# kostastsa/BayesianFiltering

Measured on AMD Instinct MI355X. Metric: filter timesteps/sec (batch x T), higher is better.
Workload: dtype f32; 1 GPU; batched Kalman filter state_dim=4 obs_dim=2 T=10000 batch=65536 per GPU, K=1, all five posterior streams (FULL5), layout=reference, observations drawn from the model; batch_per_gpu=65536, T=10000, state_dim=4, obs_dim=2, parallelism=batch-sharded x1

## Files before the change

bayesianfiltering_amd/csrc/bf_api.hip:

```cpp
#include <cstring>
#include "bf_common.hpp"
#include "../../include/bayesfilt_ext2.h"
#include "forward_host.hpp"
#include "pscan_host.hpp"
#include "user_model.hpp"
#include "bf_rng.hpp"

namespace bf {

char* last_error_buf() {
  static thread_local char buf[512] = {0};
  return buf;
}

int set_error(int code, const char* fmt, ...) {
  va_list ap;
  va_start(ap, fmt);
  vsnprintf(last_error_buf(), 512, fmt, ap);
  va_end(ap);
  return code;
}

int launch_kf_group(const bf_lgssm* p, const bf_cstream* y, long long B, long long T, const bf_carry* carry,
                    const bf_out_desc* out, hipStream_t stream, int force_mode, int lanes);
// ... 56 lines not shown
static Option g_kf_lanes{0, OPT_KF_LANES};
__host__ __device__ inline float canon_eval_one(int op, const float* in, long long n, long long i) {
  const float x = in[i];
  float s, c;
  switch (op) {
    case 0: return canon_log(x);
    case 1: return canon_exp(x);
    case 2: return bits_to_normal(canon_f_bits(x));
    case 3: canon_sincos(x, &s, &c); return s;
    case 4: canon_sincos(x, &s, &c); return c;
    default: return canon_atan2(x, in[n + i]);
  }
}
__global__ void canon_eval_kernel(int op, const float* __restrict__ in, long long n, float* __restrict__ out) {
  const long long i = (long long)blockIdx.x * blockDim.x + threadIdx.x;
  if (i >= n) return;
  out[i] = canon_eval_one(op, in, n, i);
}

Option& rts_load_mode_option();
static Option g_kf_small_mode{1, OPT_KF_SMALL_MODE};
static Option g_force_generic{0, OPT_FORCE_GENERIC};
Option& force_generic_option() { return g_force_generic; }

static bool kf_small_tiles(int n, int m) { return n >= 9 && n <= 32 && m <= 32 && (n >= 16 || m > 8) && g_kf_small_mode.load() != 0; }

struct GsfTiles {
  bool linear;
  bf_lgssm lg;
  int dyn_kind;
  float dth[8];
};
static GsfTiles gsf_tiles(const bf_model* model, int K) {
  GsfTiles t;
  std::memset(&t, 0, sizeof(t));
  const bool lin_emi = model->emi_id == 0 && model->n_emi_theta == model->m * model->n + model->m * model->dr;
  const bool lin_dyn = model->dyn_id == 0 && model->n_dyn_theta == model->n * model->n + model->n * model->dq;
  t.dyn_kind = (model->dyn_id == 1 && model->n_dyn_theta == 5 && model->dq == model->n) ? 1
             : (model->dyn_id == 4 && model->n_dyn_theta == 1 && model->dq == model->n) ? 2 : 0;
  t.linear = lin_emi && model->flags == 0 && K <= 64 && (lin_dyn || t.dyn_kind != 0);
  if (!t.linear) return t;
  bf_lgssm& lg = t.lg;
  lg.n = model->n; lg.dq = model->dq; lg.m = model->m; lg.dr = model->dr;
  if (lin_dyn) { lg.A = model->dyn_theta; lg.G = model->dyn_theta + model->n * model->n; t.dyn_kind = 0; }
  lg.H = model->emi_theta; lg.D = model->emi_theta + model->m * model->n;
  lg.q0 = model->q0; lg.r0 = model->r0; lg.Q = model->Q; lg.R = model->R;
  lg.Q_steps = model->Q_steps > 0 ? model->Q_steps : 1; lg.R_steps = model->R_steps > 0 ? model->R_steps : 1;
  if (!lin_dyn) for (int i = 0; i < model->n_dyn_theta && i < 8; ++i) t.dth[i] = model->dyn_theta[i];
  return t;
}
Option& ffbs_spl_option();
Option& pkf_block_option();
Option& prs_block_option();
Option& pfs_block_option();
long long kf_pscan_workspace_bytes(int n, int m, long long B, long long T, int block);
int launch_kf_pscan(const bf_lgssm* model, const bf_cstream* y, long long B, long long T, const bf_carry* carry,
                    const bf_out_desc* out, void* workspace, long long workspace_bytes, hipStream_t stream, bool missing);

template <class F>
static int with_generic_fallback(int rc, F&& generic) {
  if (rc != BF_EUNSUPPORTED) return rc;
  char first[512];
  std::snprintf(first, sizeof(first), "%s", last_error_buf());
  const int rc2 = generic();
  if (rc2 == BF_OK) return BF_OK;
  char second[512];
  std::snprintf(second, sizeof(second), "%s", last_error_buf());
  return set_error(rc2, "%.240s; generic kernel: %.240s", first, second);
}

}

extern "C" {

int bf_version(void) { return BF_VERSION; }

int bf_abi_check(int32_t header_version, size_t sizeof_out_desc, size_t sizeof_lgssm, size_t sizeof_model,
                 size_t sizeof_bpf_model, size_t sizeof_bpf_out) {
  if (header_version / 100 != BF_VERSION / 100)
    return bf::set_error(BF_EINVAL, "binding was written against header version %d, the library is %d", (int)header_version, BF_VERSION);
  BF_ABI_SIZE(sizeof_out_desc, bf_out_desc)
  BF_ABI_SIZE(sizeof_lgssm, bf_lgssm)
  BF_ABI_SIZE(sizeof_model, bf_model)
  BF_ABI_SIZE(sizeof_bpf_model, bf_bpf_model)
  BF_ABI_SIZE(sizeof_bpf_out, bf_bpf_out)
  return BF_OK;
}

const char* bf_last_error(void) { return bf::last_error_buf(); }

int bf_device_count(void) {
  int n = 0;
  if (hipGetDeviceCount(&n) != hipSuccess) return 0;
  int ok = 0;
  for (int i = 0; i < n; ++i) {
    hipDeviceProp_t prop;
    if (hipGetDeviceProperties(&prop, i) == hipSuccess && std::strncmp(prop.gcnArchName, "gfx950", 6) == 0) ++ok;
  }
  return ok;
}

static int set_option_impl(const char* name, int value, bool this_call_only) {
  struct Row {
    const char* name;
    bf::Option& option;
    bool (*accept)(int);
    const char* message;
  };
  const auto flag = [](int v) { return v == 0 || v == 1; };
  const auto pscan_block = [](int v) { return v == 0 || (v >= bf::PSCAN_L_MIN && v <= bf::PSCAN_L_MAX); };
  static_assert(bf::PSCAN_L_MIN == 4 && bf::PSCAN_L_MAX == 4096, "the *_block messages below spell the limits out");
  const Row rows[] = {
      {"kf_emit_mode", bf::g_kf_emit_mode, [](int v) { return v >= -1 && v <= 2; }, "kf_emit_mode must be -1..2"},
      {"kf_lanes", bf::g_kf_lanes, [](int v) { return v >= 0 && v <= 64 && (v & (v - 1)) == 0; }, "kf_lanes must be 0 or a power of two <= 64"},
      {"kf_small_mode", bf::g_kf_small_mode, flag, "kf_small_mode must be 0 or 1"},
      {"force_generic", bf::g_force_generic, flag, "force_generic must be 0 or 1"},
      {"ugsf_force_generic", bf::g_ugsf_force_generic, flag, "ugsf_force_generic must be 0 or 1"},
      {"agsf_force_generic", bf::g_agsf_force_generic, flag, "agsf_force_generic must be 0 or 1"},
      {"rts_load_mode", bf::rts_load_mode_option(), [](int v) { return v == -1 || v == 0 || v == 2; }, "rts_load_mode must be -1, 0 or 2"},
      {"ffbs_spl", bf::ffbs_spl_option(), [](int v) { return v == 0 || v == 1 || v == 2 || v == 4 || v == 8; }, "ffbs_spl must be 0, 1, 2, 4 or 8"},
      {"pkf_block", bf::pkf_block_option(), pscan_block, "pkf_block must be 0 or 4..4096"},
      {"prs_block", bf::prs_block_option(), pscan_block, "prs_block must be 0 or 4..4096"},
      {"pfs_block", bf::pfs_block_option(), pscan_block, "pfs_block must be 0 or 4..4096"},
      {"gsf_structured", bf::g_gsf_structured, flag, "gsf_structured must be 0 or 1"},
      {"bpf_variant", bf::g_bpf_variant, flag, "bpf_variant must be 0 or 1"},
      {"bpf_hbm_mode", bf::g_bpf_hbm_mode, [](int v) { return v >= 0 && v <= 2; }, "bpf_hbm_mode must be 0, 1 or 2"},
      {"bpf_arith", bf::g_bpf_arith, flag, "bpf_arith must be 0 or 1"},
      {"bpf_spec", bf::g_bpf_spec, flag, "bpf_spec must be 0 or 1"},
  };
  for (const Row& r : rows) {
    if (!name || std::strcmp(name, r.name) != 0) continue;
    if (!r.accept(value)) return bf::set_error(BF_EINVAL, "%s", r.message);
    if (this_call_only) {
      bf::CallOverrides& c = bf::call_overrides();
      c.value[r.option.id] = value;
      c.armed[r.option.id] = true;
    } else {
      r.option = value;
    }
    return BF_OK;
  }
  return bf::set_error(BF_EINVAL, "unknown option '%s'", name ? name : "(null)");
}

int bf_set_option(const char* name, int value) { return set_option_impl(name, value, false); }

int bf_set_call_option(const char* name, int value) { return set_option_impl(name, value, true); }

int64_t bf_bytes_per_step(int32_t n, int32_t m, int32_t K, const bf_out_desc* out) {
  int64_t per = 0;
  if (!out) {
    per = 1 + 2 * (int64_t)n + 2 * (int64_t)n * n;
  } else {
    if (out->weights.ptr) per += 1;
    if (out->means.ptr) per += n;
    if (out->covs.ptr) per += (int64_t)n * n;
    if (out->pred_means.ptr) per += n;
    if (out->pred_covs.ptr) per += (int64_t)n * n;
    if (out->loglik.ptr) per += 1;
  }
  int64_t once = 0;
  if (out && out->coll_mean.ptr) once += n;
  if (out && out->coll_cov.ptr) once += (int64_t)n * n;
  return 4 * (int64_t)m + 4 * (int64_t)K * per + 4 * once;
}

int bf_kalman_filter_f32(const bf_lgssm* model, const bf_cstream* y, int64_t B, int64_t T, const bf_carry* carry,
                         const bf_out_desc* out, void* stream) {
// ... 333 lines not shown
```

bayesianfiltering_amd/csrc/bf_common.hpp:

```cpp
#pragma once
#include <hip/hip_runtime.h>
#include <cstdarg>
#include <cstdio>
#include <cstdint>
#include <atomic>
#include <iterator>
#include "../../include/bayesfilt.h"
#include "bf_views.hpp"

namespace bf {

char* last_error_buf();
int set_error(int code, const char* fmt, ...);

#define BF_HIP_CHECK(expr)                                                                   \
  do {                                                                                       \
    hipError_t e_ = (expr);                                                                  \
    if (e_ != hipSuccess)                                                                    \
      return ::bf::set_error(BF_EHIP, "%s failed: %s (%s:%d)", #expr, hipGetErrorString(e_), \
                             __FILE__, __LINE__);                                            \
  } while (0)

#define BF_ABI_SIZE(NAME_, T_)           \
  if (NAME_ != 0 && NAME_ != sizeof(T_)) \
    return ::bf::set_error(BF_EINVAL, "binding's sizeof(" #T_ ") = %zu, the library's is %zu: the struct layouts differ", NAME_, sizeof(T_));

enum OptionId { OPT_KF_EMIT_MODE, OPT_KF_LANES, OPT_KF_SMALL_MODE, OPT_FORCE_GENERIC, OPT_GSF_STRUCTURED,
                OPT_BPF_VARIANT, OPT_BPF_HBM_MODE, OPT_BPF_SPEC, OPT_BPF_ARITH, OPT_RTS_LOAD_MODE, OPT_UGSF_FORCE_GENERIC, OPT_FFBS_SPL,
                OPT_AGSF_FORCE_GENERIC, OPT_PKF_BLOCK, OPT_PRS_BLOCK, OPT_PFS_BLOCK,
                OPT_COUNT };
struct CallOverrides {
  int value[OPT_COUNT];
  bool armed[OPT_COUNT];
};
CallOverrides& call_overrides();
struct Option {
  std::atomic<int> global;
  OptionId id;
  Option(int v, OptionId i) : global(v), id(i) {}
  int load() const {
    const CallOverrides& c = call_overrides();
    return c.armed[id] ? c.value[id] : global.load();
  }
  operator int() const { return load(); }
  Option& operator=(int v) {
    global = v;
    return *this;
  }
};
void begin_call_constants();
void release_call_constants();
struct CallOptionScope {
  CallOptionScope() { begin_call_constants(); }
  ~CallOptionScope() {
    CallOverrides& c = call_overrides();
    for (int i = 0; i < OPT_COUNT; ++i) c.armed[i] = false;
    release_call_constants();
  }
};

int device_constants(const void* host, size_t bytes, hipStream_t stream, const void** d_out);

#ifndef BF_MISSING
#define BF_MISSING false
#endif
#if BF_MISSING
#define BF_GROUP_FN(FAMILY_, G_) launch_##FAMILY_##_missing_group_##G_
#else
#define BF_GROUP_FN(FAMILY_, G_) launch_##FAMILY_##_group_##G_
#endif

template <class Group, class... Args>
inline int run_groups(Group* const* groups, size_t count, bool* matched, const Args&... args) {
  *matched = false;
  for (size_t g = 0; g < count; ++g) {
    const int rc = groups[g](args..., matched);
    if (*matched) return rc;
  }
  return BF_OK;
}

inline SView make_sview(const bf_stream& s) { return SView{s.ptr, s.sB, s.sK, s.sT, s.sE}; }
// ... 5 lines not shown
```

bayesianfiltering_amd/csrc/kf_scan_mfma.hip:

```cpp
#include <cstdlib>
#include "forward_host.hpp"
#include "lgssm_pack.hpp"
#include "mfma_multi.hpp"
#include "mfma_tiles.hpp"

namespace bf {

template <int N, int M>
struct MfmaConst {
  float reserved[N * N + M * N];
  float GQG[N * N], DRD[M * M], Gq0[N], Dr0[M];
  float dth[8];
  unsigned short A3[3][N * N], H3[3][M * N];
};

__device__ __attribute__((noinline)) void chol_w_rows_bf(lds_f* sc, lds_f* sT, lds_f* sv, lds_f* mcur, lds_f* mnxt, lds_f* scv, lds_c* wt,
                                                         int lane) {
  chol_w_rows_impl<64>(sc, sT, sv, mcur, mnxt, scv, wt, lane);
}
__device__ __attribute__((noinline, used)) float chol_loglik_rows(lds_f* sc, lds_f* sv, int lane) { return chol_loglik_rows_impl(sc, sv, lane); }

template <int N>
__device__ __forceinline__ void store_tile(const SView& sv, long long b, long long t, int pi, int pj, int lane, const f32x16& acc, int k = 0) {
  if (!sv.p) return;
  const int lr = lane & 31, lk = lane >> 5;
  gl_f* base = per_step(sv.p + b * sv.sB + k * sv.sK + t * sv.sT);
  const unsigned e0 = (unsigned)((32 * pi + 4 * lk) * N + 32 * pj + lr);
  if (sv.sE == 1) {
    BF_UNROLL for (int r = 0; r < 16; ++r) __builtin_nontemporal_store(acc[r], base + (e0 + ((r & 3) + 8 * (r >> 2)) * N));
  } else {
    const long long sE = sv.sE + (long long)opaque_szero();
    const unsigned e0s = e0 + (unsigned)opaque_zero();
    BF_UNROLL for (int r = 0; r < 16; ++r) __builtin_nontemporal_store(acc[r], base + (long long)(e0s + ((r & 3) + 8 * (r >> 2)) * N) * sE);
  }
}
template <int N>
__device__ __forceinline__ void store_tile_n(const SView& sv, long long b, long long t, int pi, int pj, int lane, const f32x16& acc, int nr, int k = 0) {
  if (nr == N) return store_tile<N>(sv, b, t, pi, pj, lane, acc, k);
  if (!sv.p) return;
  const int lr = lane & 31, lk = lane >> 5;
  gl_f* base = per_step(sv.p + b * sv.sB + k * sv.sK + t * sv.sT);
  const int col = 32 * pj + lr;
  const long long sE = sv.sE + (long long)opaque_szero();
  BF_UNROLL for (int r = 0; r < 16; ++r) {
    const int row = 32 * pi + (r & 3) + 8 * (r >> 2) + 4 * lk;
    if (col < nr && row < nr) __builtin_nontemporal_store(acc[r], base + (long long)(row * nr + col) * sE);
  }
}

__device__ __forceinline__ float dot_terms_half(const u32x4 (*x)[4], const float* v, int lk, int h) {
  float s = 0.f;
  BF_UNROLL for (int cc = 0; cc < 2; ++cc) BF_UNROLL for (int d = 0; d < 4; ++d) {
    const u32x4 x0v = h ? x[0][2 + cc] : x[0][cc], x1v = h ? x[1][2 + cc] : x[1][cc], x2v = h ? x[2][2 + cc] : x[2][cc];
    const float x0 = (bf_lo(x0v[d]) + bf_lo(x1v[d])) + bf_lo(x2v[d]);
    const float x1 = (bf_hi(x0v[d]) + bf_hi(x1v[d])) + bf_hi(x2v[d]);
    const int k = 16 * (2 * h + cc) + 8 * lk + 2 * d;
    s = fmaf(x0, v[k], s);
    s = fmaf(x1, v[k + 1], s);
  }
  return s;
}

template <int N, int M, bool MULTI = false, bool TV = false, int DYN = 0>
__global__ void __launch_bounds__(256, 2)
kf_scan_mfma5_kernel(const MfmaConst<N, M>* __restrict__ cst, CView y, CarryView carry, OutViews out, long long B, long long T,
                     int rot_mode, int nr, int mr, int K, const float* __restrict__ tvq, const float* __restrict__ tvr) {
  static_assert(N == 64 && M == 32, "tile assignment is written for n = 64, m = 32");
  constexpr int PS = M + 1, HPP = N + 1;
  constexpr int PITCH = 144, PN_TERM = 64 * PITCH, ZN_TERM = 32 * PITCH, WT_PITCH = 80, WT_TERM = 64 * WT_PITCH;
  constexpr int OFF_ZN = 3 * PN_TERM, OFF_WT = OFF_ZN + 3 * ZN_TERM, OFF_YN = OFF_ZN, OFF_F32 = OFF_WT + 3 * WT_TERM;
  static_assert(3 * PN_TERM <= 3 * ZN_TERM + 3 * WT_TERM, "Y^T aliases Z and W^T");
  const int tid = threadIdx.x;
  const int lane = tid & 63;
  const int lr = lane & 31, lk = lane >> 5;
  __shared__ int s_rot;
  if (tid == 0) {
    const unsigned hw = __builtin_amdgcn_s_getreg((31 << 11) | 4);
    const unsigned k = (hw >> 4) & 3, pos = ((k & 1) << 1) | (k >> 1);
    s_rot = rot_mode == 0 ? (int)blockIdx.x : (int)(pos + 2 * (hw & 15));
  }
  __syncthreads();
  const int wave = __builtin_amdgcn_readfirstlane(((tid >> 6) + s_rot) & 3);
  const int ti = wave >> 1, tj = wave & 1;
  const long long b = blockIdx.x;
  const long long bt = MULTI ? b / K : b;
  const int kc = MULTI ? (int)(b % K) : 0;

  extern __shared__ __attribute__((aligned(16))) float lds[];
  lds_c* L = (lds_c*)reinterpret_cast<char*>(lds);
  lds_c* Pn = L;
  lds_c* Zn = L + OFF_ZN;
  lds_c* Wt = L + OFF_WT;
  lds_c* Yn = L + OFF_YN;
  float* sHP = lds + OFF_F32 / 4;
  float* sc2 = sHP + M * HPP;
  float* sc3 = sc2 + M * PS;
  float* sm = sc3 + M * PS;
  float* sm2 = sm + N;
  float* sv = sm2 + N;
  float* scv = sv + M;
  float* part = scv + N;
  float* sv3 = part + 2 * N;

  u32x4 hop[3][4], aop[3][4];
  BF_UNROLL for (int t = 0; t < 3; ++t) BF_UNROLL for (int c = 0; c < 4; ++c) {
    hop[t][c] = *reinterpret_cast<const u32x4*>(&cst->H3[t][lr * N + 16 * c + 8 * lk]);
    if constexpr (DYN == 0) aop[t][c] = *reinterpret_cast<const u32x4*>(&cst->A3[t][(32 * tj + lr) * N + 16 * c + 8 * lk]);
  }
  f32x16 Pacc;
  const bool col_ok = 32 * tj + lr < nr;
  BF_UNROLL for (int r = 0; r < 16; ++r) {
    const int row = 32 * ti + c_row(r, lane);
    Pacc[r] = (col_ok && row < nr) ? carry.P_in[b * nr * nr + row * nr + 32 * tj + lr] : 0.f;
  }
  store_terms_transposed(Pn, PN_TERM, PITCH, ti, tj, lane, Pacc);
  if (tid < N) sm[tid] = tid < nr ? carry.m_in[b * nr + tid] : 0.f;
  float w = (!MULTI && carry.w_in) ? carry.w_in[b] : 1.0f;
  float ynext = (wave >= 2 && lane < mr) ? y.p[bt * y.sB + lane * y.sE] : 0.f;
  const float ll_pad = 0.5f * 1.8378770664093453f * (float)(M - mr);
  const float dr0 = cst->Dr0[lr], gq0 = cst->Gq0[lane];
  __syncthreads();

#ifdef BF_MFMA_PHASE_TIMERS
  long long tacc[12] = {0};
  long long tprev = wall_clock64();
#define BF_TICK5(i) { const long long tn_ = wall_clock64(); tacc[i] += tn_ - tprev; tprev = tn_; }
#else
#define BF_TICK5(i)
#endif
  float* mcur = sm;
  float* mnxt = sm2;
  for (long long t = 0; t < T; ++t) {
    float yv_t = ynext;
    if (wave >= 2) {
      const long long tn = t + 1 < T ? t + 1 : t;
      if (lane < mr) ynext = y.p[bt * y.sB + tn * y.sT + lane * y.sE];
    }
    gl_cf* const drd_t = TV && tvr ? per_step(tvr + t * (M * M)) : per_step(cst->DRD);
    gl_cf* const gqg_t = TV && tvq ? per_step(tvq + t * (N * N)) : per_step(cst->GQG);
    if (wave < 2) {
      f32x16 z = {0};
      BF_UNROLL for (int c = 0; c < 4; ++c) {
        u32x4 a[3];
        load_terms(a, Pn, PN_TERM, PITCH, 32 * wave + lr, c, lk);
        const u32x4 bh[3] = {hop[0][c], hop[1][c], hop[2][c]};
        z = mfma_bf6(a, bh, z);
      }
      BF_UNROLL for (int r = 0; r < 16; ++r) sHP[lr * HPP + 32 * wave + c_row(r, lane)] = z[r];
      store_terms_transposed(Zn, ZN_TERM, PITCH, wave, 0, lane, z);
    } else {
      float s = dot_terms_half(hop, mcur, lk, wave - 2);
      s += __shfl_xor(s, 32, 64);
      if (lane < M) part[(wave - 2) * N + lane] = s;
    }
    BF_TICK5(0)
    lds_barrier();
    BF_TICK5(1)
    float ll = 0.f;
    if (wave >= 2) {
      {
        if (lane < M) (wave == 2 ? sv : sv3)[lane] = yv_t - ((part[lane] + part[N + lane]) + dr0);
      }
      f32x16 acc;
      BF_UNROLL for (int r = 0; r < 16; ++r) acc[r] = drd_t[lr * M + c_row(r, lane)];
      BF_UNROLL for (int c = 0; c < 4; ++c) {
        u32x4 bz[3];
        load_terms(bz, Zn, ZN_TERM, PITCH, lr, c, lk);
        const u32x4 ah[3] = {hop[0][c], hop[1][c], hop[2][c]};
        acc = mfma_bf6(ah, bz, acc);
      }
      float* sc = wave == 2 ? sc2 : sc3;
      BF_UNROLL for (int r = 0; r < 16; ++r) sc[lr * PS + c_row(r, lane)] = acc[r];
      wave_lds_order();
      BF_TICK5(10)
      if (wave == 3) chol_w_rows_bf((lds_f*)sc3, (lds_f*)sHP, (lds_f*)sv3, (lds_f*)mcur, (lds_f*)mnxt, (lds_f*)scv, Wt, lane);
      else ll = chol_loglik_rows((lds_f*)sc2, (lds_f*)sv, lane) + ll_pad;
    }
    BF_TICK5(2)
    lds_barrier();
    BF_TICK5(3)
    {
      f32x16 acc = Pacc;
      BF_UNROLL for (int c = 0; c < 2; ++c) {
        u32x4 a[3], bw[3];
        load_terms(a, Wt, WT_TERM, WT_PITCH, 32 * ti + lr, c, lk);
        load_terms(bw, Wt, WT_TERM, WT_PITCH, 32 * tj + lr, c, lk);
        BF_UNROLL for (int q = 0; q < 3; ++q) a[q] ^= 0x80008000u;
        acc = mfma_bf6(a, bw, acc);
      }
      acc = mfma2(lk == 0 ? scv[32 * ti + lr] : 0.f, lk == 0 ? scv[32 * tj + lr] : 0.f, acc);
      store_tile_n<N>(out.P, bt, t, ti, tj, lane, acc, nr, kc);
      store_terms_transposed(Pn, PN_TERM, PITCH, ti, tj, lane, acc);
    }
    if (wave == 1 && out.m.p && lane < nr) out.m.p[bt * out.m.sB + kc * out.m.sK + t * out.m.sT + lane * out.m.sE] = mnxt[lane];
    if (wave == 2 && lane == 0) {
      if constexpr (!MULTI) {
        w = reweight_single(ll, w);
        if (out.w.p) out.w.p[b * out.w.sB + t * out.w.sT] = w;
      }
      if (out.ll.p) out.ll.p[bt * out.ll.sB + kc * out.ll.sK + t * out.ll.sT] = ll;
    }
    BF_TICK5(4)
    lds_barrier();
    BF_TICK5(5)
    float gq[16];
    BF_UNROLL for (int r = 0; r < 16; ++r) gq[r] = gqg_t[(32 * ti + c_row(r, lane)) * N + 32 * tj + lr];
    if constexpr (DYN != 0) {
      gl_cf* th = per_step(cst->dth);
      const int row = 32 * tj + lr;
      float fv = 0.f;
      BF_UNROLL for (int c = 0; c < 4; ++c) {
        float fr[8];
        BF_UNROLL for (int e = 0; e < 8; ++e) fr[e] = 0.f;
        if (row < nr) {
          if constexpr (DYN == 1) {
            const float alpha = th[0], beta = th[1], gamma = th[2], dt = th[3];
            const bool mp = th[4] != 0.f;
            const int im1 = (row + nr - 1) % nr, ip1 = (row + 1) % nr, im2 = (row + 2 * nr - 2) % nr;
            const float xi = mnxt[row], ax = mnxt[im1];
            const float bx = mp ? (mnxt[ip1] - mnxt[im2]) : 0.f;
            fv = xi + dt * (alpha * (ax * bx) - beta * xi + gamma);
            BF_UNROLL for (int e = 0; e < 8; ++e) {
              const int j = 16 * c + 8 * lk + e;
              float v = 0.f;
              if (j == row) v += 1.0f - dt * beta;
              if (mp) {
                if (j == im1) v += dt * alpha * bx;
                if (j == ip1) v += dt * alpha * ax;
                if (j == im2) v -= dt * alpha * ax;
              }
              fr[e] = v;
            }
          } else {
            const float w0 = th[0], xi = mnxt[row];
            fv = sinf(w0 * xi);
            const float d = w0 * cosf(w0 * xi);
            BF_UNROLL for (int e = 0; e < 8; ++e) fr[e] = (16 * c + 8 * lk + e == row) ? d : 0.f;
          }
        }
        BF_UNROLL for (int d = 0; d < 4; ++d) {
          const Split3 sp = split_pair(fr[2 * d], fr[2 * d + 1]);
          aop[0][c][d] = sp.hi; aop[1][c][d] = sp.mid; aop[2][c][d] = sp.lo;
        }
      }
      if (ti == 0 && lane < 32) { part[32 * tj + lane] = fv; part[N + 32 * tj + lane] = 0.f; }
    }
    {
      f32x16 acc = {0};
      BF_UNROLL for (int c = 0; c < 4; ++c) {
        u32x4 a[3];
        load_terms(a, Pn, PN_TERM, PITCH, 32 * ti + lr, c, lk);
        const u32x4 ba[3] = {aop[0][c], aop[1][c], aop[2][c]};
        acc = mfma_bf6(a, ba, acc);
      }
      store_terms_transposed(Yn, PN_TERM, PITCH, ti, tj, lane, acc);
    }
    if constexpr (DYN == 0) {
      float s = dot_terms_half(aop, mnxt, lk, ti);
      s += __shfl_xor(s, 32, 64);
      if (lane < 32) part[ti * N + 32 * tj + lane] = s;
    }
    BF_TICK5(6)
    lds_barrier();
    BF_TICK5(7)
    {
      if (wave == 2) mcur[lane] = (part[lane] + part[N + lane]) + gq0;
      BF_UNROLL for (int r = 0; r < 16; ++r) Pacc[r] = 0.f;
      BF_UNROLL for (int c = 0; c < 4; ++c) {
        u32x4 a[3];
        load_terms(a, Yn, PN_TERM, PITCH, 32 * ti + lr, c, lk);
        const u32x4 ba[3] = {aop[0][c], aop[1][c], aop[2][c]};
        Pacc = mfma_bf6(a, ba, Pacc);
      }
      BF_UNROLL for (int r = 0; r < 16; ++r) Pacc[r] += gq[r];
      store_tile_n<N>(out.pP, bt, t, ti, tj, lane, Pacc, nr, kc);
      store_terms_transposed(Pn, PN_TERM, PITCH, ti, tj, lane, Pacc);
    }
    if (wave == 2 && out.pm.p && lane < nr) out.pm.p[bt * out.pm.sB + kc * out.pm.sK + t * out.pm.sT + lane * out.pm.sE] = (part[lane] + part[N + lane]) + gq0;
    BF_TICK5(8)
    lds_barrier();
    BF_TICK5(9)
  }

  if (carry.P_out && col_ok) BF_UNROLL for (int r = 0; r < 16; ++r) {
      const int row = 32 * ti + c_row(r, lane);
      if (row < nr) carry.P_out[b * nr * nr + row * nr + 32 * tj + lr] = Pacc[r];
    }
  if (carry.m_out && tid < nr) carry.m_out[b * nr + tid] = mcur[tid];
  if (!MULTI && carry.w_out && wave == 2 && lane == 0) carry.w_out[b] = w;
#ifdef BF_MFMA_PHASE_TIMERS
  __syncthreads();
  if (b == 0 && lane == 0 && carry.P_out) for (int i = 0; i < 12; ++i) carry.P_out[wave * 16 + i] = (float)tacc[i];
#endif
}

int launch_kf_mfma(const bf_lgssm* p, const bf_cstream* y, long long B, long long T, const bf_carry* carry,
                   const bf_out_desc* out, hipStream_t stream, int K, bool multi, int dyn_kind, const float* dth) {
  constexpr int N = 64, M = 32;
  const int nr = p->n, mr = p->m, dq = p->dq, dr = p->dr;
  if (nr > N || mr > M) return set_error(BF_EUNSUPPORTED, "MFMA Kalman kernel: n <= 64 and m <= 32");
  if (dyn_kind != 0 && (!multi || p->G || dq != nr)) return set_error(BF_EINVAL, "nonlinear chains: identity noise input, multi launch");
  if (K > 64) return set_error(BF_EUNSUPPORTED, "MFMA Kalman kernel: at most 64 components (one per lane in the weight update)");
  if ((p->Q_steps > 1 && p->Q_steps != T) || (p->R_steps > 1 && p->R_steps != T))
    return set_error(BF_EINVAL, "time-varying covariances need one matrix per step (Q_steps / R_steps = T = %lld)", T);
  MfmaConst<N, M>* h = new MfmaConst<N, M>();
  for (int i = 0; i < 8; ++i) h->dth[i] = (dyn_kind != 0 && dth) ? dth[i] : 0.f;
  if (dyn_kind == 0) split_bf16x3(p->A, nr, nr, nr, h->A3, N);
  split_bf16x3(p->H, mr, nr, nr, h->H3, N);
  noise_cov(p->G, p->Q, nr, dq, h->GQG, N);
  noise_cov(p->D, p->R, mr, dr, h->DRD, M);
  for (int i = mr; i < M; ++i) h->DRD[i * M + i] = 1.0f;
  noise_mean(p->G, p->q0, nr, dq, h->Gq0);
  noise_mean(p->D, p->r0, mr, dr, h->Dr0);
  const void* dv = nullptr;
  const int crc = device_constants(h, sizeof(*h), stream, &dv);
  delete h;
  if (crc != BF_OK) return crc;
  const MfmaConst<N, M>* d = static_cast<const MfmaConst<N, M>*>(dv);

  auto [yv, cv, ov] = forward_views(y, carry, out);
  float *d_tvq = nullptr, *d_tvr = nullptr, *llscratch = nullptr;
  auto free_tables = [&]() {
    if (d_tvq) (void)hipFreeAsync(d_tvq, stream);
    if (d_tvr) (void)hipFreeAsync(d_tvr, stream);
  };
  int rc = BF_OK;
  if (p->Q_steps > 1) rc = tv_table_on_device(p->G, p->Q, T, nr, dq, N, N, stream, &d_tvq);
  if (rc == BF_OK && p->R_steps > 1) rc = tv_table_on_device(p->D, p->R, T, mr, dr, M, mr, stream, &d_tvr);
  if (rc == BF_OK && multi) rc = begin_multi(B, T, K, stream, ov, &llscratch);
  if (rc != BF_OK) { free_tables(); return rc; }

  static const int rot_mode = [] { const char* e = std::getenv("BAYESFILT_MFMA_ROT"); return e ? std::atoi(e) : 1; }();
  const size_t lds5 = 3 * 64 * 144 + 3 * 32 * 144 + 3 * 64 * 80 + sizeof(float) * (size_t)(M * (N + 1) + 2 * M * (M + 1) + 5 * N + 2 * M);
  const long long chains = multi ? B * K : B;
  auto go = [&](auto kern5) {
    const hipError_t ae = hipFuncSetAttribute(reinterpret_cast<const void*>(kern5), hipFuncAttributeMaxDynamicSharedMemorySize, (int)lds5);
    if (ae != hipSuccess) return ae;
    hipLaunchKernelGGL(kern5, dim3((unsigned)chains), dim3(256), lds5, stream, d, yv, cv, ov, chains, T, rot_mode, nr, mr, K, d_tvq, d_tvr);
    return hipGetLastError();
  };
  const bool tv = d_tvq || d_tvr;
  hipError_t le;
  if (multi && dyn_kind == 1) le = tv ? go(kf_scan_mfma5_kernel<N, M, true, true, 1>) : go(kf_scan_mfma5_kernel<N, M, true, false, 1>);
  else if (multi && dyn_kind == 2) le = tv ? go(kf_scan_mfma5_kernel<N, M, true, true, 2>) : go(kf_scan_mfma5_kernel<N, M, true, false, 2>);
  else if (multi) le = tv ? go(kf_scan_mfma5_kernel<N, M, true, true>) : go(kf_scan_mfma5_kernel<N, M, true, false>);
  else le = tv ? go(kf_scan_mfma5_kernel<N, M, false, true>) : go(kf_scan_mfma5_kernel<N, M, false, false>);
  free_tables();
  if (le != hipSuccess && llscratch) (void)hipFreeAsync(llscratch, stream);
  BF_HIP_CHECK(le);
  if (multi) return finish_multi(ov, carry, B, T, K, stream, llscratch);
  return BF_OK;
}

}
```

bayesianfiltering_amd/csrc/mfma_tiles.hpp:

```cpp
#pragma once
#include "bf_common.hpp"
#include "kf_math.hpp"
#include "lane_group.hpp"
#include "scan_common.hpp"

namespace bf {

using f32x16 = __attribute__((ext_vector_type(16))) float;
using lds_f = __attribute__((address_space(3))) float;
typedef float f32x2 __attribute__((ext_vector_type(2)));
typedef __bf16 bf16x2 __attribute__((ext_vector_type(2)));
typedef __bf16 bf16x8 __attribute__((ext_vector_type(8)));
typedef unsigned u32x2 __attribute__((ext_vector_type(2)));
typedef unsigned u32x4 __attribute__((ext_vector_type(4)));
using lds_u32x2 = __attribute__((address_space(3))) u32x2;
using lds_u32x4 = __attribute__((address_space(3))) u32x4;
using lds_c = __attribute__((address_space(3))) char;
typedef __attribute__((address_space(1))) float gl_f;
typedef const __attribute__((address_space(1))) float gl_cf;

__device__ __forceinline__ f32x16 mfma2(float a, float b, f32x16 c) {
  return __builtin_amdgcn_mfma_f32_32x32x2f32(a, b, c, 0, 0, 0);
}
__device__ __forceinline__ int c_row(int r, int lane) { return (r & 3) + 8 * (r >> 2) + 4 * (lane >> 5); }
// ... 22 lines not shown
}

__device__ __forceinline__ float rsqrt_newton(float d) {
  const float y0 = __builtin_amdgcn_rsqf(d);
  const float e0 = fmaf(-(d * y0), y0, 1.0f);
  return fmaf(0.5f * y0, e0, y0);
}

struct Split3 {
  unsigned hi, mid, lo;
};
__device__ __forceinline__ unsigned pk_bf16(float a, float b) {
  return __builtin_bit_cast(unsigned, __builtin_convertvector(f32x2{a, b}, bf16x2));
}
__device__ __forceinline__ float bf_lo(unsigned pk) { return __builtin_bit_cast(float, pk << 16); }
__device__ __forceinline__ float bf_hi(unsigned pk) { return __builtin_bit_cast(float, pk & 0xffff0000u); }
__device__ __forceinline__ Split3 split_pair(float x0, float x1) {
  Split3 o;
  o.hi = pk_bf16(x0, x1);
  const float r0 = x0 - bf_lo(o.hi), r1 = x1 - bf_hi(o.hi);
  o.mid = pk_bf16(r0, r1);
  const float q0 = r0 - bf_lo(o.mid), q1 = r1 - bf_hi(o.mid);
  o.lo = pk_bf16(q0, q1);
  return o;
}

__device__ __forceinline__ f32x16 mfma_bf6(const u32x4* a, const u32x4* b, f32x16 c) {
  auto m = [](u32x4 x, u32x4 y, f32x16 acc) {
    return __builtin_amdgcn_mfma_f32_32x32x16_bf16(__builtin_bit_cast(bf16x8, x), __builtin_bit_cast(bf16x8, y), acc, 0, 0, 0);
  };
  c = m(a[1], b[1], c);
  c = m(a[0], b[2], c);
  c = m(a[2], b[0], c);
  c = m(a[0], b[1], c);
  c = m(a[1], b[0], c);
  c = m(a[0], b[0], c);
  return c;
}
__device__ __forceinline__ void store_terms_transposed(lds_c* dst, int term_bytes, int pitch, int rt, int ct, int lane, const f32x16& acc) {
  const int lr = lane & 31, lk = lane >> 5;
  lds_c* base = dst + (32 * ct + lr) * pitch + (32 * rt + 4 * lk) * 2;
  BF_UNROLL for (int g = 0; g < 4; ++g) {
    const Split3 a = split_pair(acc[4 * g], acc[4 * g + 1]), b = split_pair(acc[4 * g + 2], acc[4 * g + 3]);
    *reinterpret_cast<lds_u32x2*>(base + 16 * g) = u32x2{a.hi, b.hi};
    *reinterpret_cast<lds_u32x2*>(base + term_bytes + 16 * g) = u32x2{a.mid, b.mid};
    *reinterpret_cast<lds_u32x2*>(base + 2 * term_bytes + 16 * g) = u32x2{a.lo, b.lo};
  }
}
__device__ __forceinline__ void load_terms(u32x4* dst, const lds_c* arr, int term_bytes, int pitch, int row, int chunk, int lk) {
  const lds_c* p = arr + row * pitch + (16 * chunk + 8 * lk) * 2;
  BF_UNROLL for (int t = 0; t < 3; ++t) dst[t] = *reinterpret_cast<const lds_u32x4*>(p + t * term_bytes);
}

#ifndef BF_MFMA_RDB
#define BF_MFMA_RDB 8
#endif
template <int NCOL = 64, bool LL = false>
__device__ __forceinline__ float chol_w_rows_impl(lds_f* sc, lds_f* sT, lds_f* sv, lds_f* mcur, lds_f* mnxt, lds_f* scv,
                                                  lds_c* wt, int lane_in) {
  constexpr int PP = NCOL + 1, PS = 33, WT_TERM_B = NCOL * 80;
  const int r = lane_in & 31;
  const int lane = NCOL == 64 ? lane_in : r;
  f32x2 aw[32];
  BF_UNROLL for (int k = 0; k < 32; ++k) aw[k] = f32x2{sc[r * PS + k] + 1e-6f, sT[k * PP + lane]};
  f32x2 rgz = f32x2{1.0f, sv[r]};
  f32x2 acc_cm = f32x2{0.f, 0.f};
  float s_gg = 0.f, s_gz = 0.f, s_zz = 0.f, rprod = 1.f;
  Split3 wsp[4];
  static_for<0, 32>([&](auto J) {
    constexpr int j = decltype(J)::value;
    const float rinv = rsqrt_newton(rdlane_u(aw[j].x, j));
    const f32x2 lw = aw[j] * rinv;
    const f32x2 gz = f32x2{rdlane_u(rgz.x, j), rdlane_u(rgz.y, j)} * rinv;
    aw[j] = lw;
    rgz = __builtin_elementwise_fma(f32x2{-lw.x, -lw.x}, gz, rgz);
    acc_cm = __builtin_elementwise_fma(f32x2{lw.y, lw.y}, gz, acc_cm);
    if constexpr (LL) {
      s_gg = fmaf(gz.x, gz.x, s_gg);
      s_gz = fmaf(gz.x, gz.y, s_gz);
      s_zz = fmaf(gz.y, gz.y, s_zz);
      rprod *= rinv;
    }
    const f32x2 ntq = -(lw * rinv);
    static_for<0, (31 - j + BF_MFMA_RDB - 1) / BF_MFMA_RDB>([&](auto Cb) {
      constexpr int k0 = j + 1 + decltype(Cb)::value * BF_MFMA_RDB;
      constexpr int nk = (32 - k0) < BF_MFMA_RDB ? (32 - k0) : BF_MFMA_RDB;
      float sb[BF_MFMA_RDB];
      static_for<0, nk>([&](auto I) { sb[decltype(I)::value] = rdlane_u(aw[k0 + decltype(I)::value].x, j); });
      __builtin_amdgcn_sched_barrier(0);
      static_for<0, nk>([&](auto I) {
        constexpr int k = k0 + decltype(I)::value;
        aw[k] = __builtin_elementwise_fma(ntq, f32x2{sb[decltype(I)::value], sb[decltype(I)::value]}, aw[k]);
      });
      __builtin_amdgcn_sched_barrier(0);
    });
    if constexpr (j & 1) {
      wsp[(j >> 1) & 3] = split_pair(aw[j - 1].y, aw[j].y);
      if constexpr ((j & 7) == 7) {
        constexpr int q = j >> 3;
        *reinterpret_cast<lds_u32x4*>(wt + 0 * WT_TERM_B + lane * 80 + q * 16) = u32x4{wsp[0].hi, wsp[1].hi, wsp[2].hi, wsp[3].hi};
        *reinterpret_cast<lds_u32x4*>(wt + 1 * WT_TERM_B + lane * 80 + q * 16) = u32x4{wsp[0].mid, wsp[1].mid, wsp[2].mid, wsp[3].mid};
        *reinterpret_cast<lds_u32x4*>(wt + 2 * WT_TERM_B + lane * 80 + q * 16) = u32x4{wsp[0].lo, wsp[1].lo, wsp[2].lo, wsp[3].lo};
      }
    }
  });
  scv[lane] = acc_cm.x * 1e-3f;
  mnxt[lane] = mcur[lane] + acc_cm.y;
  if constexpr (LL) {
    const float one_m = fmaf(-1e-6f, s_gg, 1.0f);
    const float quad = s_zz + (1e-6f * s_gz) * s_gz / one_m;
    return -0.5f * quad - 0.5f * 32.0f * 1.8378770664093453f + fast_log(rprod) - 0.5f * fast_log(one_m);
  } else {
    return 0.f;
  }
}

__device__ __forceinline__ float chol_loglik_rows_impl(lds_f* sc, lds_f* sv, int lane) {
  constexpr int PS = 33;
  const int r = lane & 31;
  f32x2 ap[16];
  BF_UNROLL for (int i = 0; i < 16; ++i) ap[i] = f32x2{sc[r * PS + 2 * i], sc[r * PS + 2 * i + 1]};
  float rz = sv[r], quad = 0.f, rprod = 1.f;
  static_for<0, 32>([&](auto J) {
    constexpr int j = decltype(J)::value;
    const float ajj = (j & 1) ? ap[j / 2].y : ap[j / 2].x;
    const float rinv = rsqrt_newton(rdlane_u(ajj, j));
    const float lj = ajj * rinv;
    const float zj = rdlane_u(rz, j) * rinv;
    rz = fmaf(-lj, zj, rz);
    quad = fmaf(zj, zj, quad);
    rprod *= rinv;
    const float nt = -(lj * rinv);
    constexpr int i_first = (j + 1) / 2;
    static_for<0, (16 - i_first + BF_MFMA_RDB / 2 - 1) / (BF_MFMA_RDB / 2)>([&](auto Cb) {
      constexpr int i0 = i_first + decltype(Cb)::value * (BF_MFMA_RDB / 2);
      constexpr int ni = (16 - i0) < BF_MFMA_RDB / 2 ? (16 - i0) : BF_MFMA_RDB / 2;
      f32x2 sb[BF_MFMA_RDB / 2];
      static_for<0, ni>([&](auto I) {
        constexpr int i = i0 + decltype(I)::value;
        sb[decltype(I)::value] = f32x2{rdlane_u(ap[i].x, j), rdlane_u(ap[i].y, j)};
      });
      __builtin_amdgcn_sched_barrier(0);
      static_for<0, ni>([&](auto I) {
        constexpr int i = i0 + decltype(I)::value;
        ap[i] = __builtin_elementwise_fma(f32x2{nt, nt}, sb[decltype(I)::value], ap[i]);
      });
      __builtin_amdgcn_sched_barrier(0);
    });
  });
  return -0.5f * quad - 0.5f * 32.0f * 1.8378770664093453f + fast_log(rprod);
}

}
```

Measured before the change: 34.76 billion timesteps/s.

## Share covariance recursion across batch when priors and model are identical

```diff
diff --git a/bayesianfiltering_amd/csrc/bf_api.hip b/bayesianfiltering_amd/csrc/bf_api.hip
--- a/bayesianfiltering_amd/csrc/bf_api.hip
+++ b/bayesianfiltering_amd/csrc/bf_api.hip
@@ -132,6 +132,7 @@
 Option& ffbs_spl_option();
 Option& pkf_block_option();
 Option& prs_block_option();
+Option& kf_shared_cov_option();
 Option& pfs_block_option();
 long long kf_pscan_workspace_bytes(int n, int m, long long B, long long T, int block);
 int launch_kf_pscan(const bf_lgssm* model, const bf_cstream* y, long long B, long long T, const bf_carry* carry,
@@ -194,6 +195,7 @@
       {"kf_emit_mode", bf::g_kf_emit_mode, [](int v) { return v >= -1 && v <= 2; }, "kf_emit_mode must be -1..2"},
       {"kf_lanes", bf::g_kf_lanes, [](int v) { return v >= 0 && v <= 64 && (v & (v - 1)) == 0; }, "kf_lanes must be 0 or a power of two <= 64"},
       {"kf_small_mode", bf::g_kf_small_mode, flag, "kf_small_mode must be 0 or 1"},
+      {"kf_shared_cov", bf::kf_shared_cov_option(), flag, "kf_shared_cov must be 0 or 1"},
       {"force_generic", bf::g_force_generic, flag, "force_generic must be 0 or 1"},
       {"ugsf_force_generic", bf::g_ugsf_force_generic, flag, "ugsf_force_generic must be 0 or 1"},
       {"agsf_force_generic", bf::g_agsf_force_generic, flag, "agsf_force_generic must be 0 or 1"},
diff --git a/bayesianfiltering_amd/csrc/bf_common.hpp b/bayesianfiltering_amd/csrc/bf_common.hpp
--- a/bayesianfiltering_amd/csrc/bf_common.hpp
+++ b/bayesianfiltering_amd/csrc/bf_common.hpp
@@ -27,7 +27,7 @@
 
 enum OptionId { OPT_KF_EMIT_MODE, OPT_KF_LANES, OPT_KF_SMALL_MODE, OPT_FORCE_GENERIC, OPT_GSF_STRUCTURED,
                 OPT_BPF_VARIANT, OPT_BPF_HBM_MODE, OPT_BPF_SPEC, OPT_BPF_ARITH, OPT_RTS_LOAD_MODE, OPT_UGSF_FORCE_GENERIC, OPT_FFBS_SPL,
-                OPT_AGSF_FORCE_GENERIC, OPT_PKF_BLOCK, OPT_PRS_BLOCK, OPT_PFS_BLOCK,
+                OPT_AGSF_FORCE_GENERIC, OPT_PKF_BLOCK, OPT_PRS_BLOCK, OPT_PFS_BLOCK, OPT_KF_SHARED_COV,
                 OPT_COUNT };
 struct CallOverrides {
   int value[OPT_COUNT];
diff --git a/bayesianfiltering_amd/csrc/kf_scan_mfma.hip b/bayesianfiltering_amd/csrc/kf_scan_mfma.hip
--- a/bayesianfiltering_amd/csrc/kf_scan_mfma.hip
+++ b/bayesianfiltering_amd/csrc/kf_scan_mfma.hip
@@ -3,8 +3,12 @@
 #include "lgssm_pack.hpp"
 #include "mfma_multi.hpp"
 #include "mfma_tiles.hpp"
+#include "kf_scan_shared.hpp"
 
 namespace bf {
+
+static Option g_kf_shared_cov{1, OPT_KF_SHARED_COV};
+Option& kf_shared_cov_option() { return g_kf_shared_cov; }
 
 template <int N, int M>
 struct MfmaConst {
@@ -19,6 +23,13 @@
   chol_w_rows_impl<64>(sc, sT, sv, mcur, mnxt, scv, wt, lane);
 }
 __device__ __attribute__((noinline, used)) float chol_loglik_rows(lds_f* sc, lds_f* sv, int lane) { return chol_loglik_rows_impl(sc, sv, lane); }
+__device__ __attribute__((noinline)) void chol_w_rows_bf_tape(lds_f* sc, lds_f* sT, lds_f* sv, lds_f* mcur, lds_f* mnxt, lds_f* scv, lds_c* wt,
+                                                              int lane, float* tape) {
+  chol_w_rows_impl<64, false, true>(sc, sT, sv, mcur, mnxt, scv, wt, lane, tape);
+}
+__device__ __attribute__((noinline)) float chol_loglik_rows_tape(lds_f* sc, lds_f* sv, int lane, float* tape) {
+  return chol_loglik_rows_impl<true>(sc, sv, lane, tape);
+}
 
 template <int N>
 __device__ __forceinline__ void store_tile(const SView& sv, long long b, long long t, int pi, int pj, int lane, const f32x16& acc, int k = 0) {
@@ -61,7 +72,7 @@
   return s;
 }
 
-template <int N, int M, bool MULTI = false, bool TV = false, int DYN = 0>
+template <int N, int M, bool MULTI = false, bool TV = false, int DYN = 0, int SHARED = 0>
 __global__ void __launch_bounds__(256, 2)
 kf_scan_mfma5_kernel(const MfmaConst<N, M>* __restrict__ cst, CView y, CarryView carry, OutViews out, long long B, long long T,
                      int rot_mode, int nr, int mr, int K, const float* __restrict__ tvq, const float* __restrict__ tvr) {
@@ -70,6 +81,10 @@
   constexpr int PITCH = 144, PN_TERM = 64 * PITCH, ZN_TERM = 32 * PITCH, WT_PITCH = 80, WT_TERM = 64 * WT_PITCH;
   constexpr int OFF_ZN = 3 * PN_TERM, OFF_WT = OFF_ZN + 3 * ZN_TERM, OFF_YN = OFF_ZN, OFF_F32 = OFF_WT + 3 * WT_TERM;
   static_assert(3 * PN_TERM <= 3 * ZN_TERM + 3 * WT_TERM, "Y^T aliases Z and W^T");
+  static_assert(SHARED == 0 || (!MULTI && !TV && DYN == 0), "the shared route: one linear model, constant Q and R");
+  if constexpr (SHARED != 0) {
+    if ((*reinterpret_cast<const unsigned*>(tvq) != 0u) == (SHARED == 1)) return;
+  }
   const int tid = threadIdx.x;
   const int lane = tid & 63;
   const int lr = lane & 31, lk = lane >> 5;
@@ -173,8 +188,14 @@
       BF_UNROLL for (int r = 0; r < 16; ++r) sc[lr * PS + c_row(r, lane)] = acc[r];
       wave_lds_order();
       BF_TICK5(10)
-      if (wave == 3) chol_w_rows_bf((lds_f*)sc3, (lds_f*)sHP, (lds_f*)sv3, (lds_f*)mcur, (lds_f*)mnxt, (lds_f*)scv, Wt, lane);
-      else ll = chol_loglik_rows((lds_f*)sc2, (lds_f*)sv, lane) + ll_pad;
+      if constexpr (SHARED == 1) {
+        float* const tape = const_cast<float*>(tvq) + SC_WS_HEAD + t * sc_step_floats(nr);
+        if (wave == 3) chol_w_rows_bf_tape((lds_f*)sc3, (lds_f*)sHP, (lds_f*)sv3, (lds_f*)mcur, (lds_f*)mnxt, (lds_f*)scv, Wt, lane, tape);
+        else ll = chol_loglik_rows_tape((lds_f*)sc2, (lds_f*)sv, lane, tape) + ll_pad;
+      } else {
+        if (wave == 3) chol_w_rows_bf((lds_f*)sc3, (lds_f*)sHP, (lds_f*)sv3, (lds_f*)mcur, (lds_f*)mnxt, (lds_f*)scv, Wt, lane);
+        else ll = chol_loglik_rows((lds_f*)sc2, (lds_f*)sv, lane) + ll_pad;
+      }
     }
     BF_TICK5(2)
     lds_barrier();
@@ -190,6 +211,7 @@
       }
       acc = mfma2(lk == 0 ? scv[32 * ti + lr] : 0.f, lk == 0 ? scv[32 * tj + lr] : 0.f, acc);
       store_tile_n<N>(out.P, bt, t, ti, tj, lane, acc, nr, kc);
+      if constexpr (SHARED == 1) tape_tile(const_cast<float*>(tvq) + SC_WS_HEAD + t * sc_step_floats(nr) + SC_HEAD, ti, tj, lane, acc, nr);
       store_terms_transposed(Pn, PN_TERM, PITCH, ti, tj, lane, acc);
     }
     if (wave == 1 && out.m.p && lane < nr) out.m.p[bt * out.m.sB + kc * out.m.sK + t * out.m.sT + lane * out.m.sE] = mnxt[lane];
@@ -274,6 +296,7 @@
       }
       BF_UNROLL for (int r = 0; r < 16; ++r) Pacc[r] += gq[r];
       store_tile_n<N>(out.pP, bt, t, ti, tj, lane, Pacc, nr, kc);
+      if constexpr (SHARED == 1) tape_tile(const_cast<float*>(tvq) + SC_WS_HEAD + t * sc_step_floats(nr) + SC_HEAD + sc_tile_floats(nr), ti, tj, lane, Pacc, nr);
       store_terms_transposed(Pn, PN_TERM, PITCH, ti, tj, lane, Pacc);
     }
     if (wave == 2 && out.pm.p && lane < nr) out.pm.p[bt * out.pm.sB + kc * out.pm.sK + t * out.pm.sT + lane * out.pm.sE] = (part[lane] + part[N + lane]) + gq0;
@@ -341,6 +364,40 @@
   };
   const bool tv = d_tvq || d_tvr;
   hipError_t le;
+  const long long ws_bytes = (long long)sizeof(float) * (SC_WS_HEAD + T * sc_step_floats(nr));
+  if (!multi && dyn_kind == 0 && !tv && B > 1 && ws_bytes <= SC_TAPE_MAX_BYTES && g_kf_shared_cov.load() != 0) {
+    float* ws = nullptr;
+    BF_HIP_CHECK(hipMallocAsync(reinterpret_cast<void**>(&ws), (size_t)ws_bytes, stream));
+    le = hipMemsetAsync(ws, 0, sizeof(float) * SC_WS_HEAD, stream);
+    if (le == hipSuccess) {
+      const long long groups = B - 1 < 2048 ? B - 1 : 2048;
+      hipLaunchKernelGGL(prior_differs_kernel, dim3((unsigned)groups), dim3(256), 0, stream, reinterpret_cast<const unsigned*>(cv.P_in), B,
+                         nr * nr, reinterpret_cast<unsigned*>(ws));
+      le = hipGetLastError();
+    }
+    auto go_ws = [&](auto kern5, long long grid) {
+      const hipError_t ae = hipFuncSetAttribute(reinterpret_cast<const void*>(kern5), hipFuncAttributeMaxDynamicSharedMemorySize, (int)lds5);
+      if (ae != hipSuccess) return ae;
+      hipLaunchKernelGGL(kern5, dim3((unsigned)grid), dim3(256), lds5, stream, d, yv, cv, ov, B, T, rot_mode, nr, mr, K, (const float*)ws,
+                         (const float*)nullptr);
+      return hipGetLastError();
+    };
+    if (le == hipSuccess) le = go_ws(kf_scan_mfma5_kernel<N, M, false, false, 0, 1>, 1);
+    if (le == hipSuccess) {
+      const size_t ldsf = sizeof(float) * (size_t)(2 * SC_HEAD + SC_G * 2 * N);
+      const long long groups = (B - 1 + SC_G - 1) / SC_G;
+      auto follow = kf_shared_follow_kernel<MfmaConst<N, M>, SC_G>;
+      le = hipFuncSetAttribute(reinterpret_cast<const void*>(follow), hipFuncAttributeMaxDynamicSharedMemorySize, (int)ldsf);
+      if (le == hipSuccess) {
+        hipLaunchKernelGGL(follow, dim3((unsigned)groups), dim3(64 * SC_G), ldsf, stream, d, yv, cv, ov, B, T, nr, mr, (const float*)ws);
+        le = hipGetLastError();
+      }
+    }
+    if (le == hipSuccess) le = go_ws(kf_scan_mfma5_kernel<N, M, false, false, 0, 2>, B);
+    (void)hipFreeAsync(ws, stream);
+    BF_HIP_CHECK(le);
+    return BF_OK;
+  }
   if (multi && dyn_kind == 1) le = tv ? go(kf_scan_mfma5_kernel<N, M, true, true, 1>) : go(kf_scan_mfma5_kernel<N, M, true, false, 1>);
   else if (multi && dyn_kind == 2) le = tv ? go(kf_scan_mfma5_kernel<N, M, true, true, 2>) : go(kf_scan_mfma5_kernel<N, M, true, false, 2>);
   else if (multi) le = tv ? go(kf_scan_mfma5_kernel<N, M, true, true>) : go(kf_scan_mfma5_kernel<N, M, true, false>);
diff --git a/bayesianfiltering_amd/csrc/kf_scan_shared.hpp b/bayesianfiltering_amd/csrc/kf_scan_shared.hpp
--- /dev/null
+++ b/bayesianfiltering_amd/csrc/kf_scan_shared.hpp
@@ -0,0 +1,178 @@
+#pragma once
+#include "mfma_tiles.hpp"
+
+namespace bf {
+
+typedef float f32x4 __attribute__((ext_vector_type(4)));
+
+constexpr int SC_WS_HEAD = 64;
+constexpr int SC_G = 8;
+constexpr long long SC_TAPE_MAX_BYTES = 512ll << 20;
+__host__ __device__ inline long long sc_tile_floats(int nr) { return (long long)((nr * nr + 3) & ~3); }
+__host__ __device__ inline long long sc_step_floats(int nr) { return SC_HEAD + 2 * sc_tile_floats(nr); }
+
+__global__ void __launch_bounds__(256) prior_differs_kernel(const unsigned* __restrict__ P, long long B, int nn, unsigned* __restrict__ flag) {
+  unsigned diff = 0u;
+  for (int e = threadIdx.x; e < nn; e += 256) {
+    const unsigned ref = P[e];
+    _Pragma("unroll 8") for (long long b = 1 + blockIdx.x; b < B; b += gridDim.x) diff |= P[b * nn + e] ^ ref;
+  }
+  if (__builtin_amdgcn_ballot_w64(diff != 0u) != 0ull && (threadIdx.x & 63) == 0) atomicOr(flag, 1u);
+}
+
+__device__ __forceinline__ void tape_tile(float* dst, int pi, int pj, int lane, const f32x16& acc, int nr) {
+  const int col = 32 * pj + (lane & 31);
+  BF_UNROLL for (int r = 0; r < 16; ++r) {
+    const int row = 32 * pi + c_row(r, lane);
+    if (col < nr && row < nr) dst[row * nr + col] = acc[r];
+  }
+}
+
+template <int G>
+__device__ __forceinline__ void copy_tile(const float* __restrict__ src, float* dst, long long sB, long long sE, int nn, int cnt, int tid) {
+  const bool wide = sE == 1 && (nn & 3) == 0 && (sB & 3) == 0 && (reinterpret_cast<unsigned long long>(dst) & 15ull) == 0ull;
+  if (wide) {
+    for (int i = tid; i < (nn >> 2); i += 64 * G) {
+      const f32x4 v = reinterpret_cast<const f32x4*>(src)[i];
+      BF_UNROLL for (int g = 0; g < G; ++g)
+        if (g < cnt) __builtin_nontemporal_store(v, reinterpret_cast<f32x4*>(dst + g * sB) + i);
+    }
+  } else {
+    for (int e = tid; e < nn; e += 64 * G) {
+      const float v = src[e];
+      BF_UNROLL for (int g = 0; g < G; ++g)
+        if (g < cnt) __builtin_nontemporal_store(v, dst + g * sB + e * sE);
+    }
+  }
+}
+
+template <class CST, int G>
+__global__ void __launch_bounds__(64 * G)
+kf_shared_follow_kernel(const CST* __restrict__ cst, CView y, CarryView carry, OutViews out, long long B, long long T, int nr, int mr,
+                        const float* __restrict__ ws) {
+#pragma clang fp contract(off)
+  constexpr int N = 64, M = 32;
+  if (*reinterpret_cast<const unsigned*>(ws) != 0u) return;
+  const int tid = threadIdx.x, lane = tid & 63, lr = lane & 31, lk = lane >> 5;
+  const int wv = __builtin_amdgcn_readfirstlane(tid >> 6);
+  const long long b0 = 1 + (long long)blockIdx.x * G;
+  const int cnt = (int)(B - b0 < G ? B - b0 : G);
+  const bool live = wv < cnt;
+  const long long b = live ? b0 + wv : b0;
+  const int nn = nr * nr;
+  const long long step = sc_step_floats(nr), tile = sc_tile_floats(nr);
+  const float* const tape = ws + SC_WS_HEAD;
+
+  extern __shared__ __attribute__((aligned(16))) float lds[];
+  float* const head = lds;
+  float* const sm = lds + 2 * SC_HEAD + wv * (2 * N);
+  float* const sm2 = sm + N;
+
+  float hrow[32], arow[64];
+  BF_UNROLL for (int c = 0; c < 4; ++c) {
+    u32x4 x[3];
+    BF_UNROLL for (int q = 0; q < 3; ++q) x[q] = *reinterpret_cast<const u32x4*>(&cst->H3[q][lr * N + 16 * c + 8 * lk]);
+    BF_UNROLL for (int d = 0; d < 4; ++d) {
+      hrow[8 * c + 2 * d] = (bf_lo(x[0][d]) + bf_lo(x[1][d])) + bf_lo(x[2][d]);
+      hrow[8 * c + 2 * d + 1] = (bf_hi(x[0][d]) + bf_hi(x[1][d])) + bf_hi(x[2][d]);
+    }
+  }
+  BF_UNROLL for (int c = 0; c < 8; ++c) {
+    u32x4 x[3];
+    BF_UNROLL for (int q = 0; q < 3; ++q) x[q] = *reinterpret_cast<const u32x4*>(&cst->A3[q][lane * N + 8 * c]);
+    BF_UNROLL for (int d = 0; d < 4; ++d) {
+      arow[8 * c + 2 * d] = (bf_lo(x[0][d]) + bf_lo(x[1][d])) + bf_lo(x[2][d]);
+      arow[8 * c + 2 * d + 1] = (bf_hi(x[0][d]) + bf_hi(x[1][d])) + bf_hi(x[2][d]);
+    }
+  }
+  const float dr0 = cst->Dr0[lr], gq0 = cst->Gq0[lane];
+  const float ll_pad = 0.5f * 1.8378770664093453f * (float)(M - mr);
+  float mminus = lane < nr ? carry.m_in[b * nr + lane] : 0.f;
+  float w = carry.w_in ? carry.w_in[b] : 1.0f;
+  float ynext = lr < mr ? y.p[b * y.sB + lr * y.sE] : 0.f;
+  sm[lane] = mminus;
+  constexpr int HEAD4 = SC_HEAD / 4, HLD = (HEAD4 + 64 * G - 1) / (64 * G);
+  BF_UNROLL for (int i = 0; i < HLD; ++i)
+    if (tid + 64 * G * i < HEAD4) reinterpret_cast<f32x4*>(head)[tid + 64 * G * i] = reinterpret_cast<const f32x4*>(tape)[tid + 64 * G * i];
+
+  for (long long t = 0; t < T; ++t) {
+    __syncthreads();
+    const float* const tp = head + (t & 1) * SC_HEAD;
+    const float* const tstep = tape + t * step;
+    f32x4 nxt[HLD];
+    if (t + 1 < T) {
+      BF_UNROLL for (int i = 0; i < HLD; ++i)
+        if (tid + 64 * G * i < HEAD4) nxt[i] = reinterpret_cast<const f32x4*>(tstep + step)[tid + 64 * G * i];
+    }
+    const float yv = ynext;
+    {
+      const long long tn = t + 1 < T ? t + 1 : t;
+      if (lr < mr) ynext = y.p[b * y.sB + tn * y.sT + lr * y.sE];
+    }
+    if (out.P.p) copy_tile<G>(tstep + SC_HEAD, out.P.p + b0 * out.P.sB + t * out.P.sT, out.P.sB, out.P.sE, nn, cnt, tid);
+    if (out.pP.p) copy_tile<G>(tstep + SC_HEAD + tile, out.pP.p + b0 * out.pP.sB + t * out.pP.sT, out.pP.sB, out.pP.sE, nn, cnt, tid);
+    float v;
+    {
+      float sh[2];
+      BF_UNROLL for (int h = 0; h < 2; ++h) {
+        float s = 0.f;
+        BF_UNROLL for (int cc = 0; cc < 2; ++cc) BF_UNROLL for (int e = 0; e < 8; ++e)
+          s = fmaf(hrow[8 * (2 * h + cc) + e], sm[16 * (2 * h + cc) + 8 * lk + e], s);
+        s += __shfl_xor(s, 32, 64);
+        sh[h] = s;
+      }
+      v = yv - ((sh[0] + sh[1]) + dr0);
+    }
+    float rz = v, rz2 = v, acc = 0.f, quad = 0.f;
+    BF_UNROLL for (int j = 0; j < 32; ++j) {
+      const float zj = rdlane_u(rz, j) * tp[SC_RINV + j];
+      rz = fmaf(-tp[SC_LW + 32 * j + lr], zj, rz);
+      acc = fmaf(tp[SC_W + 64 * j + lane], zj, acc);
+      const float z2 = rdlane_u(rz2, j) * tp[SC_RINV2 + j];
+      rz2 = fmaf(-tp[SC_L2 + 32 * j + lr], z2, rz2);
+      quad = fmaf(z2, z2, quad);
+    }
+    const float mplus = mminus + acc;
+    const float ll = loglik_of_chain(quad, tp[SC_RPROD]) + ll_pad;
+    w = reweight_single(ll, w);
+    sm2[lane] = mplus;
+    wave_lds_order();
+    {
+      float ph[2];
+      BF_UNROLL for (int h = 0; h < 2; ++h) {
+        float s2[2];
+        BF_UNROLL for (int kk = 0; kk < 2; ++kk) {
+          float s = 0.f;
+          BF_UNROLL for (int cc = 0; cc < 2; ++cc) BF_UNROLL for (int e = 0; e < 8; ++e)
+            s = fmaf(arow[16 * (2 * h + cc) + 8 * kk + e], sm2[16 * (2 * h + cc) + 8 * kk + e], s);
+          s2[kk] = s;
+        }
+        ph[h] = s2[0] + s2[1];
+      }
+      mminus = (ph[0] + ph[1]) + gq0;
+    }
+    sm[lane] = mminus;
+    wave_lds_order();
+    if (live) {
+      if (out.m.p && lane < nr) out.m.p[b * out.m.sB + t * out.m.sT + lane * out.m.sE] = mplus;
+      if (out.pm.p && lane < nr) out.pm.p[b * out.pm.sB + t * out.pm.sT + lane * out.pm.sE] = mminus;
+      if (lane == 0) {
+        if (out.w.p) out.w.p[b * out.w.sB + t * out.w.sT] = w;
+        if (out.ll.p) out.ll.p[b * out.ll.sB + t * out.ll.sT] = ll;
+      }
+    }
+    if (t + 1 < T) {
+      f32x4* const dst = reinterpret_cast<f32x4*>(head + ((t + 1) & 1) * SC_HEAD);
+      BF_UNROLL for (int i = 0; i < HLD; ++i)
+        if (tid + 64 * G * i < HEAD4) dst[tid + 64 * G * i] = nxt[i];
+    }
+  }
+
+  if (carry.P_out) copy_tile<G>(tape + (T - 1) * step + SC_HEAD + tile, carry.P_out + b0 * nn, nn, 1, nn, cnt, tid);
+  if (live) {
+    if (carry.m_out && lane < nr) carry.m_out[b * nr + lane] = mminus;
+    if (carry.w_out && lane == 0) carry.w_out[b] = w;
+  }
+}
+
+}
diff --git a/bayesianfiltering_amd/csrc/mfma_tiles.hpp b/bayesianfiltering_amd/csrc/mfma_tiles.hpp
--- a/bayesianfiltering_amd/csrc/mfma_tiles.hpp
+++ b/bayesianfiltering_amd/csrc/mfma_tiles.hpp
@@ -98,12 +98,27 @@
   BF_UNROLL for (int t = 0; t < 3; ++t) dst[t] = *reinterpret_cast<const lds_u32x4*>(p + t * term_bytes);
 }
 
+constexpr int SC_LW = 0;
+constexpr int SC_W = 1024;
+constexpr int SC_L2 = 3072;
+constexpr int SC_RINV = 4096;
+constexpr int SC_RINV2 = 4128;
+constexpr int SC_RPROD = 4160;
+constexpr int SC_HEAD = 4164;
+
+__device__ __forceinline__ float loglik_of_chain(float quad, float rprod) {
+#pragma clang fp contract(off)
+  const float lg = __builtin_amdgcn_logf(rprod) * 0.6931471805599453f;
+  const float head = -0.5f * quad - 0.5f * 32.0f * 1.8378770664093453f;
+  return head + lg;
+}
+
 #ifndef BF_MFMA_RDB
 #define BF_MFMA_RDB 8
 #endif
-template <int NCOL = 64, bool LL = false>
+template <int NCOL = 64, bool LL = false, bool TAPE = false>
 __device__ __forceinline__ float chol_w_rows_impl(lds_f* sc, lds_f* sT, lds_f* sv, lds_f* mcur, lds_f* mnxt, lds_f* scv,
-                                                  lds_c* wt, int lane_in) {
+                                                  lds_c* wt, int lane_in, float* tape = nullptr) {
   constexpr int PP = NCOL + 1, PS = 33, WT_TERM_B = NCOL * 80;
   const int r = lane_in & 31;
   const int lane = NCOL == 64 ? lane_in : r;
@@ -119,6 +134,11 @@
     const f32x2 lw = aw[j] * rinv;
     const f32x2 gz = f32x2{rdlane_u(rgz.x, j), rdlane_u(rgz.y, j)} * rinv;
     aw[j] = lw;
+    if constexpr (TAPE) {
+      if (lane_in < 32) tape[SC_LW + 32 * j + lane_in] = lw.x;
+      tape[SC_W + 64 * j + lane_in] = lw.y;
+      if (lane_in == 0) tape[SC_RINV + j] = rinv;
+    }
     rgz = __builtin_elementwise_fma(f32x2{-lw.x, -lw.x}, gz, rgz);
     acc_cm = __builtin_elementwise_fma(f32x2{lw.y, lw.y}, gz, acc_cm);
     if constexpr (LL) {
@@ -161,7 +181,8 @@
   }
 }
 
-__device__ __forceinline__ float chol_loglik_rows_impl(lds_f* sc, lds_f* sv, int lane) {
+template <bool TAPE = false>
+__device__ __forceinline__ float chol_loglik_rows_impl(lds_f* sc, lds_f* sv, int lane, float* tape = nullptr) {
   constexpr int PS = 33;
   const int r = lane & 31;
   f32x2 ap[16];
@@ -173,6 +194,10 @@
     const float rinv = rsqrt_newton(rdlane_u(ajj, j));
     const float lj = ajj * rinv;
     const float zj = rdlane_u(rz, j) * rinv;
+    if constexpr (TAPE) {
+      if (lane < 32) tape[SC_L2 + 32 * j + lane] = lj;
+      if (lane == 0) tape[SC_RINV2 + j] = rinv;
+    }
     rz = fmaf(-lj, zj, rz);
     quad = fmaf(zj, zj, quad);
     rprod *= rinv;
@@ -194,6 +219,10 @@
       __builtin_amdgcn_sched_barrier(0);
     });
   });
+  if constexpr (TAPE) {
+    if (lane == 0) tape[SC_RPROD] = rprod;
+    return loglik_of_chain(quad, rprod);
+  }
   return -0.5f * quad - 0.5f * 32.0f * 1.8378770664093453f + fast_log(rprod);
 }
 
```

New measurement: 34.80 billion timesteps/s, median of 2. No clear change (+0.1%).
